# haoyann/koordinator

Measured on AMD Instinct MI355X. Metric: pod-node Filter+Score evals/sec + p99 per-pod sched latency @50k nodes, higher is better.
Workload: dtype int64

## Files before the change

### include/koord_eval.h

```cpp
#ifndef KOORD_EVAL_H
#define KOORD_EVAL_H

#include <stdint.h>

#ifdef __cplusplus
extern "C" {
#endif

#define KE_ABI_VERSION 14
#define KE_ABSENT (-1)

typedef struct ke_ctx ke_ctx;

#define KE_OK 0
#define KE_ERR_INVALID (-1)
#define KE_ERR_UNSUPPORTED (-2)
#define KE_ERR_DEVICE (-3)
#define KE_ERR_NOT_FOUND (-4)
#define KE_ERR_NO_DEVICE (-5)

#define KE_CODE_SUCCESS 0
#define KE_CODE_ERROR 1
#define KE_CODE_UNSCHEDULABLE 2
#define KE_CODE_UNSCHEDULABLE_AND_UNRESOLVABLE 3
// ... 656 lines not shown
int ke_last_kernel_stats(ke_ctx* ctx, double* eval_ms, double* select_ms, double* resolve_ms, int32_t* samples);
int ke_last_kernel_stats_ex(ke_ctx* ctx, double* v8, int32_t* samples, int32_t* pipelined_batches);
int ke_set_pipeline(ke_ctx* ctx, int32_t on);
int ke_last_host_stats(ke_ctx* ctx, double* ms8);
int ke_last_resolve_split(ke_ctx* ctx, double* prologue_ms, double* replay_ms);
int ke_debug_resolve_phases(ke_ctx* ctx, double* phases6);
int ke_debug_resolve_subphases(ke_ctx* ctx, double* sub5);
int ke_debug_resolve_wave1(ke_ctx* ctx, double* w4);
int ke_debug_numa_deferred(ke_ctx* ctx, int64_t* n);
int ke_debug_ds_cuts(ke_ctx* ctx, int32_t* cuts);
int ke_debug_rsv_fused(ke_ctx* ctx, int64_t* out2);
int ke_debug_replay_phases(ke_ctx* ctx, double* cyc8);
int ke_debug_kernel_phases(ke_ctx* ctx, int32_t kernel, double* cyc8);
int ke_debug_spec_failed(ke_ctx* ctx, double* per_batch);
int ke_debug_call_boundary(ke_ctx* ctx, int64_t* out4);
int ke_debug_check_records(ke_ctx* ctx, int64_t now_ns, int64_t* mismatched_nodes);
int ke_bench_eval_kernel(ke_ctx* ctx, int32_t n_pods, const ke_pod* pods, int64_t now_ns, int32_t iters,
                         double* avg_ms);

int ke_row_bytes(void);
int ke_pod_record_bytes(void);
int ke_debug_rows(ke_ctx* ctx, int32_t n, int64_t now_ns, void* device_rows, void* host_rows);
int64_t ke_debug_usage_bound(int64_t total, int64_t thr);
int32_t ke_num_nodes(ke_ctx* ctx);
int ke_debug_node_state(ke_ctx* ctx, int32_t node, ke_node* out, int32_t cpu_cap, ke_cpu* cpus, int32_t* n_cpus,
                        int32_t zone_cap, ke_numa_zone* zones, int32_t* n_zones, int32_t dev_cap, ke_device* devs,
                        int32_t* n_devs);

#ifdef __cplusplus
}
// ... 3 lines not shown
```

### koordinator_amd/abi.py

```python
import ctypes as C
import os

import numpy as np

ABI_VERSION = 14
ABSENT = -1

OK = 0
ERR_INVALID, ERR_UNSUPPORTED, ERR_DEVICE, ERR_NOT_FOUND, ERR_NO_DEVICE = -1, -2, -3, -4, -5

CODE_SUCCESS, CODE_ERROR, CODE_UNSCHEDULABLE, CODE_UNSCHEDULABLE_AND_UNRESOLVABLE, CODE_SKIP = 0, 1, 2, 3, 5

REASON_NONE = 0
REASON_LA_NODEMETRIC_EXPIRED = 1
REASON_LA_USAGE_CPU = 2
REASON_LA_USAGE_MEMORY = 3
REASON_LA_AGG_USAGE_CPU = 4
REASON_LA_AGG_USAGE_MEMORY = 5
REASON_NUMA_INSUFFICIENT_AMPLIFIED_CPU = 16
REASON_NUMA_INVALID_AMPLIFICATION_RATIO = 17
REASON_NUMA_INVALID_CPU_TOPOLOGY = 18
REASON_NUMA_POLICY_CONFLICT = 19
REASON_NUMA_MISSING_RESOURCES = 20
REASON_NUMA_HINT_UNALIGNED = 21
# ... 542 lines not shown
    "ke_last_kernel_stats_ex": (C.c_int, [C.c_void_p, C.c_void_p, C.POINTER(i32), C.POINTER(i32)]),
    "ke_set_pipeline": (C.c_int, [C.c_void_p, i32]),
    "ke_debug_replay_phases": (C.c_int, [C.c_void_p, C.c_void_p]),
    "ke_debug_kernel_phases": (C.c_int, [C.c_void_p, C.c_int32, C.c_void_p]),
    "ke_debug_check_records": (C.c_int, [C.c_void_p, i64, C.POINTER(i64)]),
    "ke_last_host_stats": (C.c_int, [C.c_void_p, C.c_void_p]),
    "ke_last_resolve_split": (C.c_int, [C.c_void_p, C.POINTER(C.c_double), C.POINTER(C.c_double)]),
    "ke_debug_resolve_phases": (C.c_int, [C.c_void_p, C.c_void_p]),
    "ke_debug_resolve_subphases": (C.c_int, [C.c_void_p, C.c_void_p]),
    "ke_debug_resolve_wave1": (C.c_int, [C.c_void_p, C.c_void_p]),
    "ke_debug_numa_deferred": (C.c_int, [C.c_void_p, C.POINTER(i64)]),
    "ke_debug_ds_cuts": (C.c_int, [C.c_void_p, C.POINTER(i32)]),
    "ke_debug_rsv_fused": (C.c_int, [C.c_void_p, C.POINTER(i64)]),
    "ke_debug_spec_failed": (C.c_int, [C.c_void_p, C.POINTER(C.c_double)]),
    "ke_debug_call_boundary": (C.c_int, [C.c_void_p, C.c_void_p]),
    "ke_bench_eval_kernel": (C.c_int, [C.c_void_p, i32, C.c_void_p, i64, i32, C.POINTER(C.c_double)]),
    "ke_row_bytes": (C.c_int, []),
    "ke_pod_record_bytes": (C.c_int, []),
    "ke_debug_rows": (C.c_int, [C.c_void_p, i32, i64, C.c_void_p, C.c_void_p]),
    "ke_debug_usage_bound": (i64, [i64, i64]),
    "ke_num_nodes": (i32, [C.c_void_p]),
    "ke_debug_node_state": (C.c_int, [C.c_void_p, i32, C.c_void_p, i32, C.c_void_p, C.c_void_p, i32, C.c_void_p,
                                      C.c_void_p, i32, C.c_void_p, C.c_void_p]),
    "ke_comm_unique_id": (C.c_int, [C.c_void_p, i32]),
    "ke_shard_init": (C.c_int, [C.c_void_p, i32, i32, C.c_void_p]),
    "ke_shard_init_host": (C.c_int, [C.c_void_p, i32, i32, C.c_void_p, C.c_void_p]),
    "ke_shard_range": (C.c_int, [C.c_void_p, C.POINTER(i32), C.POINTER(i32)]),
}
COMM_ID_BYTES = 128

_lib = None


def load_library(path=LIB_PATH):
    global _lib
    if _lib is not None and path == LIB_PATH:
        return _lib
    if not os.path.exists(path):
        raise RuntimeError(f"{path} is missing: run __graft_entry__.build() (hipcc --offload-arch=gfx950)")
    lib = C.CDLL(path)
    for name, (res, args) in EXPORTS.items():
        fn = getattr(lib, name)
        fn.restype = res
        fn.argtypes = args
    if lib.ke_abi_version() != ABI_VERSION:
        raise RuntimeError("libkoordeval.so ABI version mismatch")
    sizes = (i32 * len(STRUCTS))()
    lib.ke_abi_struct_sizes(sizes, len(STRUCTS))
    for s, n in zip(STRUCTS, sizes):
        if C.sizeof(s) != n:
            raise RuntimeError(f"ABI layout mismatch for {s.__name__}: python {C.sizeof(s)} != C {n}")
    if path == LIB_PATH:
        _lib = lib
    return lib


def ptr(arr):
# ... 17 lines not shown
```

### koordinator_amd/csrc/ke_capi.cpp

```cpp
#include <algorithm>
#include <chrono>
#include <cstring>
#include <deque>
#include <new>

#include "ke_host.h"

namespace ke {
const char* last_error_cstr();
int device_available();
int device_create(Context* ctx);
void device_destroy(Context* ctx);
int device_eval(Context* ctx, int32_t n_pods, const ke_pod* pods, int64_t now, uint8_t* status, uint8_t* reason,
                int16_t* la, int16_t* numa, int16_t* ds, int16_t* total, int32_t* best);
int device_schedule(Context* ctx, int32_t n_pods, const ke_pod* pods, int64_t now, int32_t* chosen, int32_t* score);
int device_rsv_result(Context* ctx, int32_t* out4);
int device_rsv_gate(const Context* ctx);
int device_refresh(Context* ctx, int64_t now, bool defer);
int device_ds_views(Context* ctx, const ke_pod& pod, int64_t now, const std::vector<DsView>& views,
                    std::vector<DsViewOut>& out);
int device_rsv_views(Context* ctx, const ke_pod& pod, int64_t now, const std::vector<RsvView>& views,
                     std::vector<RsvViewOut>& out);
int device_numa_views(Context* ctx, const ke_pod& pod, int64_t now, const std::vector<NumaRsvView>& views,
                      std::vector<NumaRsvOut>& out);
// ... 1534 lines not shown
  return device_replay_phases(&ctx->c, kernel, cyc8);
}

int ke_debug_spec_failed(ke_ctx* ctx, double* per_batch) {
  if (!ctx || !per_batch) return fail(KE_ERR_INVALID, "ke_debug_spec_failed arguments");
  *per_batch = ctx->c.kstat_spec_failed;
  return KE_OK;
}

int ke_debug_call_boundary(ke_ctx* ctx, int64_t* out4) {
  if (!ctx || !out4) return fail(KE_ERR_INVALID, "ke_debug_call_boundary arguments");
  for (int i = 0; i < 4; i++) out4[i] = ctx->c.call_boundary[i];
  return KE_OK;
}

int ke_debug_check_records(ke_ctx* ctx, int64_t now_ns, int64_t* mismatched_nodes) {
  if (ctx) async_drain(ctx);
  if (!ctx || !mismatched_nodes) return fail(KE_ERR_INVALID, "ke_debug_check_records arguments");
  flush_mirror(ctx->c);
  int rc = require_device(ctx);
  if (rc) return rc;
  return device_check_records(&ctx->c, now_ns, mismatched_nodes);
}

int ke_set_pipeline(ke_ctx* ctx, int32_t on) {
  if (ctx) async_drain(ctx);
  if (!ctx) return fail(KE_ERR_INVALID, "null context");
  int rc = require_device(ctx);
  if (rc) return rc;
  return device_set_pipeline(&ctx->c, on);
// ... 121 lines not shown
```

### koordinator_amd/csrc/ke_host.h

```cpp
#pragma once
#include <atomic>
#include <chrono>
#include <cstdint>
#include <functional>
#include <map>
#include <string>
#include <thread>
#include <utility>
#include <vector>

#include "../../include/koord_eval.h"
#include "ke_types.h"

namespace ke {

struct AssignedPod {
  struct {
    int64_t pod_key;
    int64_t custom_seconds_after_scheduled, custom_seconds_after_initialized, initialized_transition_ns;
    int32_t priority_class;
    uint8_t has_initialized;
  } pod;
  int64_t ts;
  int64_t est[KE_NRES];
// ... 85 lines not shown
  bool ext_enabled = false;
  int32_t n_bind_nodes = 0;
  int32_t n_policy_nodes = 0;
  std::vector<uint64_t> last_cpusets;
  std::vector<int64_t> last_numa_alloc;
  std::vector<uint64_t> last_dev_alloc;
  std::vector<int32_t> last_chosen;
  std::vector<int64_t> last_uid;
  std::vector<uint8_t> last_quota;
  DeviceState* dev = nullptr;
  double last_total_ms = 0.0;
  std::vector<double> last_batch_ms;
  double kstat_eval_ms = 0, kstat_select_ms = 0, kstat_resolve_ms = 0, kstat_fixup_ms = 0, kstat_handoff_ms = 0;
  int32_t last_pipelined = 0;
  int64_t call_boundary[4] = {0, 0, 0, 0};
  bool call_behind = false;
  uint64_t prev_end_tick = 0;
  int32_t last_ds_cuts = 0;
  double kstat_spec_failed = 0;
  double kstat_rows_fetched = 0, kstat_rows_changed = 0;
  double last_enqueue_ms = 0;
  double host_ms[8] = {0, 0, 0, 0, 0, 0, 0, 0};
  double kstat_resolve_prologue_ms = 0, kstat_resolve_loop_ms = 0;
  double kstat_resolve_phase_ms[6] = {0, 0, 0, 0, 0, 0};
  double kstat_resolve_sub_ms[5] = {0, 0, 0, 0, 0};
  double kstat_resolve_wave1_ms[4] = {0, 0, 0, 0};
  int64_t kstat_numa_deferred = 0;
  int32_t kstat_samples = 0;
  struct PendingAssign {
    int32_t node;
// ... 171 lines not shown
```

### koordinator_amd/csrc/ke_kernels.hip

```cpp
#include <hip/hip_runtime.h>
#include <rccl/rccl.h>

#include <algorithm>
#include <chrono>
#include <cstdio>
#include <cstdlib>
#include <cstring>
#include <vector>

#include "ke_cpuacc.h"
#include "ke_merge.h"
#include "ke_host.h"
#include "ke_types.h"

namespace ke {

extern "C" __device__ uint32_t __ockl_wfred_max_u32(uint32_t);
extern "C" __device__ int32_t __ockl_wfred_add_i32(int32_t);

#define HIP_OK(expr)                                                                 \
  do {                                                                               \
    hipError_t _e = (expr);                                                          \
    if (_e != hipSuccess) {                                                          \
      return fail(KE_ERR_DEVICE, std::string(#expr ": ") + hipGetErrorString(_e));  \
    }                                                                                \
  } while (0)

constexpr int EVAL_BLOCK = 256;
constexpr int PST = 16;
inline dim3 eval_grid(int n_nodes, int block, int pods, int ppb) {
  const int tiles = (n_nodes + block - 1) / block;
  return dim3((unsigned)((tiles + 7) / 8 * 8), (unsigned)((pods + ppb - 1) / ppb));
}
constexpr int SELECT_BLOCK = 1024;
constexpr int SELECT_WAVES = SELECT_BLOCK / 64;
constexpr int KMAX = MAX_BATCH;

struct SoA {
  int64_t* f;
  uint32_t* flags;
  int64_t stride;
  int64_t* ds;
  uint64_t* dsm;
// ... 2584 lines not shown
  for (int u = 0; u < RW_PAD; u++) w[u] = __hip_atomic_load(const_cast<int64_t*>(rec + u), __ATOMIC_RELAXED, SCOPE);
  w[RW_PAD] = 0;
  rec_unpack(w, f);
}
__device__ __forceinline__ void rec_load_plain(const int64_t* __restrict__ rec, NodeFast& f) {
  int64_t w[NUM_RW];
  const int4* r4 = reinterpret_cast<const int4*>(rec);
#pragma unroll
  for (int u = 0; u < NUM_RW / 2; u++) {
    const int4 q = r4[u];
    w[2 * u] = (int64_t)(((uint64_t)(uint32_t)q.y << 32) | (uint32_t)q.x);
    w[2 * u + 1] = (int64_t)(((uint64_t)(uint32_t)q.w << 32) | (uint32_t)q.z);
  }
  rec_unpack(w, f);
}
__device__ __forceinline__ void rec_unpack(const int64_t (&w)[NUM_RW], NodeFast& f) {
#pragma unroll
  for (int v = 0; v < 2; v++)
#pragma unroll
    for (int q = 0; q < 2; q++) {
      f.fh[v][q] = w[RW_FH + 2 * v + q];
      f.sa[v][q] = __longlong_as_double(w[RW_SA + 2 * v + q]);
    }
#pragma unroll
  for (int q = 0; q < 2; q++) {
    f.cap[q] = __longlong_as_double(w[RW_CAP + q]);
    f.rcap[q] = __longlong_as_double(w[RW_RCAP + q]);
    f.al[q] = __longlong_as_double(w[RW_AL + q]);
    f.ral[q] = __longlong_as_double(w[RW_RAL + q]);
    f.nreq[q] = __longlong_as_double(w[RW_NREQ + q]);
// ... 299 lines not shown
      if ((threadIdx.x & 63) == 0 && m) atomicMax(dsmax1 + p, m);
    } else if (DS) {
      dsraw[(int64_t)p * score_stride + i] = (uint16_t)(o.total >= 0 ? 1u : 0u);
    }
    if (CPU && NUMA) aff_out[i] = o.aff;
  }
}

constexpr int EVAL_PPB = 8;
__host__ __device__ constexpr bool use_record_eval(int pods) { return pods > 2; }
template <bool EXT, int NS = 0>
__global__ __launch_bounds__(EVAL_BLOCK) void k_eval_plain(SoA s, int lo, int hi, const DevPod* __restrict__ pods,
                                                           const int32_t* __restrict__ batch_base, int batch_pods,
                                                           KArgs k, uint16_t* __restrict__ scores, int64_t score_stride,
                                                           uint64_t* __restrict__ stamp, const int32_t* __restrict__ done_wait,
                                                           int32_t* __restrict__ err) {
  if (done_wait) {
    __shared__ int32_t s_go;
    if (threadIdx.x == 0) s_go = wait_at_least(done_wait, 1, err);
    __syncthreads();
    if (!s_go) return;
  }
  if (stamp && (blockIdx.x | blockIdx.y | threadIdx.x) == 0) stamp[0] = __builtin_amdgcn_s_memrealtime();
  const int G = (int)gridDim.y;
  const int b = (int)(blockIdx.x + blockIdx.y * gridDim.x), r = b >> 3;
  const int tile = (r / G) * 8 + (b & 7), group = r % G;
  const int i = lo + tile * blockDim.x + threadIdx.x;
  const int base = *batch_base;
  const int p0 = group * EVAL_PPB;
  const int np = min(batch_pods, p0 + EVAL_PPB) - p0;
  __shared__ double s_pd[EVAL_PPB][4];
  __shared__ int64_t s_pi[EVAL_PPB][3];
  __shared__ uint32_t s_pf[EVAL_PPB];
  __shared__ uint64_t s_ns[NS ? EVAL_PPB : 1][EVAL_BLOCK / 64];
  uint64_t off[2] = {0ull, 0ull};
  if constexpr (NS == NS_SCORES) {
    static_assert(EVAL_PPB == 8, "two words of four offsets");
#pragma unroll
    for (int q = 0; q < EVAL_PPB; q++) {
      const uint16_t v = q < np && i < hi ? s.nsc_tbl[(int64_t)((uint32_t)s.ns_ids[base + p0 + q] >> 16) * s.nsc_stride + i] : (uint16_t)0;
      off[q >> 2] |= (uint64_t)v << ((q & 3) * 16);
    }
  }
  if ((int)threadIdx.x < 4 * np) {
    const int q = threadIdx.x >> 2, c = threadIdx.x & 3;
    const DevPod& pp = pods[base + p0 + q];
    if constexpr (NS) {
      static_assert(EVAL_BLOCK / 64 == 4, "one table word per wave of the block");
      const int w = ((lo + tile * (int)blockDim.x) >> 6) + c;
      const int idw = s.ns_ids[base + p0 + q];
      s_ns[q][c] = w < s.ns_wps ? s.ns_tbl[(int64_t)(NS == NS_SCORES ? idw & 0xffff : idw) * s.ns_wps + w] : 0ull;
    }
    s_pd[q][c] = (double)(c < 2 ? pp.est[c] : pp.req[c - 2]);
    if (!EXT && c < 3) s_pi[q][c] = c < 2 ? pp.est[c] : pp.req[0];
    if (!EXT && c == 3) s_pf[q] = pp.flags;
  }
  __syncthreads();
  if (i >= hi) return;
  NodeFast f;
  rec_load_plain(s.rec + (int64_t)i * NUM_RW, f);
  if (EXT && (k.flags & AF_EXT)) ext_load(s, i, k, f);
  fast_adopt(f, k);
  uint16_t* const out = scores + (int64_t)p0 * score_stride + i;
  for (int q = 0; q < np; q++) {
    const double ed[2] = {s_pd[q][0], s_pd[q][1]}, rd[2] = {s_pd[q][2], s_pd[q][3]};
    int32_t t;
    if constexpr (EXT) {
      t = fast_total<EXT>(f, pods[base + p0 + q], ed, rd, k);
    } else {
      DevPod pl;
      pl.flags = s_pf[q];
      pl.est[0] = s_pi[q][0];
      pl.est[1] = s_pi[q][1];
      pl.req[0] = s_pi[q][2];
      t = fast_total<false>(f, pl, ed, rd, k);
    }
    if constexpr (NS == NS_SCORES) t = t >= 0 ? t + (int32_t)((uint32_t)((q < 4 ? off[0] : off[1]) >> ((q & 3) * 16)) & 0xffffu) : t;
    if (NS && !((s_ns[q][threadIdx.x >> 6] >> (threadIdx.x & 63)) & 1ull)) t = -1;
    out[(int64_t)q * score_stride] = (uint16_t)(t + 1);
  }
}

template <bool EXT, int NS = 0>
__global__ __launch_bounds__(64) void k_patch(SoA s, const DevPod* __restrict__ pods, const int32_t* __restrict__ batch_base,
                                              KArgs k, const int32_t* __restrict__ tlist, uint16_t* __restrict__ scores,
                                              int64_t score_stride, const int32_t* __restrict__ done_wait,
                                              int32_t* __restrict__ err) {
  const int j = blockIdx.x, t = threadIdx.x;
  {
    __shared__ int32_t s_go;
    if (t == 0) s_go = wait_at_least(done_wait, 1, err);
    __syncthreads();
    if (!s_go) return;
  }
  const int n = ld_sc1(tlist);
// ... 3194 lines not shown
    int64_t cpusets_cap = 0;
    int32_t* d_sched = nullptr;
    int64_t sched_cap = 0;
    PinnedVec<uint8_t> h_out;
    std::vector<hipEvent_t> tev;
  } alt;
  uint16_t* d_scores2 = nullptr;
  uint32_t* d_split2 = nullptr;
  uint32_t* d_stale = nullptr;
  uint32_t* d_pre = nullptr;
  uint32_t* d_chg = nullptr;
  int64_t* d_trows = nullptr;
  int32_t* d_tcnt = nullptr;
  int32_t* d_parts_done = nullptr;
  int32_t* d_stale_cnt = nullptr;
  static constexpr int EV_RING = 8;
  hipEvent_t ev_res[EV_RING] = {};
  hipEvent_t ev_sel[EV_RING] = {};
  hipEvent_t ev_start = nullptr;
  hipEvent_t ev_refresh[2] = {};
  bool refresh_pending[2] = {};
  int refresh_cur = 0;
  std::vector<std::function<void(const int32_t*)>> deferred;
  int32_t* d_rsv_gate = nullptr;
  bool refresh_sync = false;
  bool pipeline = true;
  bool pipe_fixup = false;
  unsigned excl_lds = EXCL_LDS;
  bool eval_patch = true;
  bool select_ahead = true;
// ... 83 lines not shown
  HIP_OK(hipMalloc(&d->d_cand, sizeof(uint32_t) * MAX_BATCH * KMAX));
  HIP_OK(hipMalloc(&d->d_cand_cnt, sizeof(int32_t) * MAX_BATCH));
  HIP_OK(hipMalloc(&d->d_batch_base, sizeof(int32_t)));
  HIP_OK(hipMemsetAsync(d->d_batch_base, 0, sizeof(int32_t), d->stream));
  HIP_OK(hipMalloc(&d->d_stale, sizeof(uint32_t) * 2 * MAX_BATCH * KSTALE));
  HIP_OK(hipMalloc(&d->d_pre, sizeof(uint32_t) * 2 * MAX_BATCH * (KSTALE2 + 1)));
  HIP_OK(hipMalloc(&d->d_stale_cnt, sizeof(int32_t) * 2 * MAX_BATCH));
  HIP_OK(hipMalloc(&d->d_trows, sizeof(int64_t) * MAX_BATCH * NUM_RW));
  HIP_OK(hipMalloc(&d->soa.rec, sizeof(int64_t) * NUM_RW * d->capacity));
  HIP_OK(hipMalloc(&d->soa.kerr, sizeof(int32_t)));
  HIP_OK(hipMemsetAsync(d->soa.kerr, 0, sizeof(int32_t), d->stream));
  HIP_OK(hipMemsetAsync(d->soa.rec, 0, sizeof(int64_t) * NUM_RW * d->capacity, d->stream));
  HIP_OK(hipMalloc(&d->d_tcnt, sizeof(int32_t)));
  HIP_OK(hipMalloc(&d->d_parts_done, sizeof(int32_t) * 2 * MAX_BATCH));
  HIP_OK(hipMemset(d->d_parts_done, 0, sizeof(int32_t) * 2 * MAX_BATCH));
  if (d->capacity > (int64_t)CHG_LDS_WORDS * 32) {
    HIP_OK(hipMalloc(&d->d_chg, sizeof(uint32_t) * (d->capacity + 31) / 32));
    HIP_OK(hipMemsetAsync(d->d_chg, 0, sizeof(uint32_t) * (d->capacity + 31) / 32, d->stream));
  }
  HIP_OK(hipMalloc(&d->d_dsraw, sizeof(uint16_t) * MAX_BATCH * d->capacity));
  HIP_OK(hipMalloc(&d->d_dsmax, sizeof(uint32_t) * DSB_WORDS));
  d->soa.dsb = d->d_dsmax;
  d->soa.dsraw = d->d_dsraw;
  HIP_OK(hipMalloc(&d->d_aff, d->capacity));
  HIP_OK(hipMalloc(&d->d_split, sizeof(uint32_t) * GATH_WORDS_MAX * MAX_WORLD));
  HIP_OK(hipMalloc(&d->d_rsv_out, sizeof(int32_t) * 4));
  HIP_OK(hipMalloc(&d->d_rsv_st, sizeof(RsvPickSt)));
  HIP_OK(hipStreamSynchronize(d->stream));
  return KE_OK;
}

int device_refresh(Context* ctx, int64_t now, bool defer = false);
int device_refresh_flush(Context* ctx, const int32_t* gate);
static KArgs make_kargs(const Context* ctx, int64_t now);
int device_rsv_views(Context* ctx, const ke_pod& pod, int64_t now, const std::vector<RsvView>& views,
                     std::vector<RsvViewOut>& out) {
  DeviceState* d = ctx->dev;
  out.assign(views.size(), RsvViewOut{});
  if (views.empty()) return KE_OK;
  HIP_OK(hipSetDevice(d->device));
  int rc = device_refresh(ctx, now);
  if (rc) return rc;
  for (const RsvView& v : views)
    if (v.node < 0 || v.node >= ctx->n_nodes) return fail(KE_ERR_DEVICE, "reservation view node out of range");
// ... 80 lines not shown
  return d->h_rsv_out.size() >= 5 ? d->h_rsv_out[4] : 0;
}

void device_destroy(Context* ctx) {
  DeviceState* d = ctx->dev;
  if (!d) return;
  (void)hipSetDevice(d->device);
  if (d->stream) (void)hipStreamSynchronize(d->stream);
  if (d->comm) (void)ncclCommDestroy(d->comm);
  void* ptrs[] = {d->soa.f,     d->soa.flags, d->d_rows,      d->d_idx,          d->d_pods,   d->d_scores,
                  d->d_cand,    d->d_cand_cnt, d->d_batch_base, d->d_out,
                  d->d_parity, d->d_best,      d->d_gath,    d->d_split,         d->soa.ds,   d->soa.dsm,
                  d->d_dsraw,   d->d_dsmax,  d->d_devalloc,   d->d_dsrows,       d->soa.nf,   d->soa.nm,
                  d->d_numaalloc, d->d_numarows, d->d_defer, d->d_defer_cnt, d->soa.cs, d->soa.cpu,
                  d->d_cpurows, d->d_cpusets, d->d_aff, d->soa.qt, d->soa.qm, d->d_sched, d->d_stale,
                  d->d_stale_cnt, d->d_pre, d->d_trows, d->d_tcnt, d->d_parts_done, d->d_scores2, d->d_split2, d->d_chg, d->soa.rec, d->soa.pt, d->soa.kerr,
                  d->soa.xf, d->soa.xm, d->d_xrows, d->soa.dsx, d->d_ph, d->d_vfo, d->d_rsv, d->d_rsv_out, d->d_rsv_st,
                  d->d_rsv_views, d->d_ds_views, d->d_numa_views, d->d_rovr, d->d_rsv_gate, d->d_ns_tbl, d->d_nsc_tbl};
  if (d->estream) (void)hipStreamSynchronize(d->estream);
  if (d->estream2) (void)hipStreamSynchronize(d->estream2);
  for (void* p : ptrs)
    if (p) (void)hipFree(p);
  for (int e = 0; e < DeviceState::EV_RING; e++) {
    if (d->ev_res[e]) (void)hipEventDestroy(d->ev_res[e]);
    if (d->ev_sel[e]) (void)hipEventDestroy(d->ev_sel[e]);
  }
  if (d->ev_start) (void)hipEventDestroy(d->ev_start);
  for (hipEvent_t e : d->ev_refresh)
    if (e) (void)hipEventDestroy(e);
  if (d->estream) (void)hipStreamDestroy(d->estream);
  if (d->cstream) (void)hipStreamDestroy(d->cstream);
// ... 1012 lines not shown
                        ? (cpu ? (numa ? k_eval_batch<true, true, true, false, true> : k_eval_batch<true, false, true, false, true>)
                               : (numa ? k_eval_batch<true, true, false, false, true> : k_eval_batch<true, false, false, false, true>))
                  : cpu ? (ds ? (numa ? k_eval_batch<true, true, true> : k_eval_batch<true, false, true>)
                              : (numa ? k_eval_batch<false, true, true> : k_eval_batch<false, false, true>))
                        : ds ? (numa ? k_eval_batch<true, true, false> : k_eval_batch<true, false, false>)
                             : (numa ? k_eval_batch<false, true, false>
                                     : ns == NS_SCORES
                                         ? ((k.flags & AF_EXT) ? k_eval_batch<false, false, false, true, false, NS_SCORES>
                                                               : k_eval_batch<false, false, false, false, false, NS_SCORES>)
                                     : ns ? ((k.flags & AF_EXT) ? k_eval_batch<false, false, false, true, false, NS_SETS>
                                                                : k_eval_batch<false, false, false, false, false, NS_SETS>)
                                          : ((k.flags & AF_EXT) ? k_eval_batch<false, false, false, true>
                                                                : k_eval_batch<false, false, false>));
        uint32_t* dcnt = numa ? d->d_defer_cnt + b : nullptr;
        if (plain_rec)
          hipLaunchKernelGGL((ns == NS_SCORES ? ((k.flags & AF_EXT) ? k_eval_plain<true, NS_SCORES> : k_eval_plain<false, NS_SCORES>)
                              : ns ? ((k.flags & AF_EXT) ? k_eval_plain<true, NS_SETS> : k_eval_plain<false, NS_SETS>)
                                 : ((k.flags & AF_EXT) ? k_eval_plain<true> : k_eval_plain<false>)), grid, dim3(eb), 0, es, d->soa,
                             lo, hi, d->d_pods, bbase, bp, k, scores, d->capacity, fold_begin ? estamps + b : nullptr,
                             wait_kernel ? nullptr : dwait, d_err);
        else
          hipLaunchKernelGGL(eval, grid, dim3(eb), 0, es, d->soa, lo, hi, d->d_pods, bbase, bp,
                             ppb, k, scores, d->capacity, d->d_dsraw, d->d_defer, dcnt, d->d_aff, d->d_dsmax,
                             fold_begin ? estamps + b : nullptr);
        if (numa) {
          uint32_t* fb = reinterpret_cast<uint32_t*>(d->d_defer + (int64_t)MAX_BATCH * d->capacity);
          hipLaunchKernelGGL((cpu ? k_numa_fallback<false, true> : k_numa_fallback<false, false>), dim3(FALLBACK_BLOCKS),
                             dim3(64), 0, es, d->soa, d->d_pods,
                             bbase, k, d->d_defer, dcnt, scores, d->capacity, 0, nullptr, nullptr,
                             nullptr, nullptr, nullptr, nullptr, ds ? d->d_dsmax : nullptr, cpu ? d->d_aff : nullptr,
                             ds ? d->d_dsraw : nullptr, fb);
          hipLaunchKernelGGL((cpu ? k_numa_finish<false, true> : k_numa_finish<false, false>), dim3(FINISH_BLOCKS),
                             dim3(64), 0, es, d->soa, d->d_pods,
                             bbase, k, d->d_defer, dcnt, scores, d->capacity, 0, nullptr, nullptr,
                             nullptr, nullptr, nullptr, nullptr, ds ? d->d_dsmax : nullptr, cpu ? d->d_aff : nullptr,
// ... 338 lines not shown
  }
  std::memcpy(&herr, h + o_err, 4);
  std::memcpy(&kerr, h + o_kerr, 4);
  const uint64_t prev_end = ctx->prev_end_tick;
  ctx->prev_end_tick = 0;
  std::memcpy(fst.data(), h + o_fst, 16 * nb);
  std::memcpy(st.data(), h + o_st, 8 * (nb + 1));
  std::memcpy(pst.data(), h + o_pst, 8 * PST * nb);
  std::memcpy(est.data(), h + o_est, 8 * nb);
  ctx->host_ms[5] = ms_since(tp);
  tp = clk::now();
  if (herr) {
    if (d->d_chg)
      (void)hipMemset(d->d_chg, 0, sizeof(uint32_t) * (d->capacity + 31) / 32);
    (void)hipMemset(d->d_parts_done, 0, sizeof(int32_t) * 2 * MAX_BATCH);
    return fail(KE_ERR_DEVICE, "pipelined schedule: a device-side hand-off timed out (placements invalid)");
  }
  if (kerr & (KERR_HINT_ROUTE | KERR_LDS_WAIT)) {
    return fail(KE_ERR_DEVICE, (kerr & KERR_LDS_WAIT) ? "internal: a replay LDS wait expired (placements invalid)"
                                                      : "internal: a hinted pod reached a kernel without the hint path");
  }
  float ms = 0;
  HIP_OK(hipEventElapsedTime(&ms, e0, e1));
  ctx->last_total_ms = ms;
  ctx->last_pipelined = n_pipelined;
  const double span = (double)(st[n_batches] - st[0]);
  const double ms_per_tick = span > 0 ? ms / span : 1e-5;
  ctx->call_boundary[0] = 0;
  ctx->call_boundary[1] = cb_copies;
  ctx->call_boundary[2] = cb_fills;
// ... 149 lines not shown
  DeviceState* d = ctx->dev;
  HIP_OK(hipSetDevice(d->device));
  if (n_pods < 1 || n_pods > MAX_BATCH || iters < 1) return fail(KE_ERR_INVALID, "bench: 1 <= n_pods <= 64, iters >= 1");
  int rc = device_refresh(ctx, now);
  if (rc) return rc;
  rc = upload_pods(ctx, n_pods, pods);
  if (rc) return rc;
  const int N = ctx->n_nodes;
  if (N == 0) return fail(KE_ERR_INVALID, "bench: no nodes");
  const KArgs k = make_kargs(ctx, now);
  const int ppb = EVAL_PPB;
  HIP_OK(hipMemsetAsync(d->d_batch_base, 0, sizeof(int32_t), d->stream));
  const dim3 grid = eval_grid(N, EVAL_BLOCK, n_pods, ppb);
  auto launch = [&]() {
    if (use_record_eval(n_pods))
      hipLaunchKernelGGL((k_eval_plain<false>), grid, dim3(EVAL_BLOCK), 0, d->stream, d->soa, 0, N, d->d_pods,
                         d->d_batch_base, n_pods, k, d->d_scores, d->capacity, nullptr, nullptr, nullptr);
    else
      hipLaunchKernelGGL((k_eval_batch<false, false, false>), grid, dim3(EVAL_BLOCK), 0, d->stream, d->soa, 0, N,
                         d->d_pods, d->d_batch_base, n_pods, ppb, k, d->d_scores, d->capacity, d->d_dsraw, d->d_defer,
                         nullptr, d->d_aff, d->d_dsmax, nullptr);
  };
  launch();
  hipEvent_t e0, e1;
  HIP_OK(hipEventCreate(&e0));
  HIP_OK(hipEventCreate(&e1));
  HIP_OK(hipEventRecord(e0, d->stream));
  for (int it = 0; it < iters; it++) launch();
  HIP_OK(hipGetLastError());
  HIP_OK(hipEventRecord(e1, d->stream));
  HIP_OK(hipEventSynchronize(e1));
  float ms = 0;
// ... 55 lines not shown
```

### koordinator_amd/csrc/ke_types.h

```cpp
#pragma once
#include <stdint.h>

#if defined(__HIPCC__) || defined(__HIP__)
#define KE_HD __host__ __device__
#else
#define KE_HD
#endif

namespace ke {

enum RowField : int {
  F_UT = 0,
  F_FH = 1,
  F_SA = 5,
  F_CAP = 9,
  F_NALLOC = 11,
  F_NREQ = 13,
  F_CSM = 15,
  F_CSAF = 16,
  F_CSAS = 17,
  NUM_I64_FIELDS = 18
};

enum NodeFlag : uint32_t {
// ... 306 lines not shown
constexpr int XF_ALLOC = 0, XF_REQ = NUM_XS, XF_PODS = 2 * NUM_XS, NUM_XF = 2 * NUM_XS + 1;

constexpr uint32_t KEY_IDX_BITS = 22;
constexpr uint32_t KEY_IDX_MASK = (1u << KEY_IDX_BITS) - 1;
constexpr int MAX_SHARD_NODES = (1 << KEY_IDX_BITS) - 1;
constexpr int MAX_TOTAL_SCORE = 1022;
constexpr int MAX_DS_RAW = 300;
KE_HD inline uint32_t make_key(int32_t total, int32_t idx) {
  return total < 0 ? 0u : ((uint32_t)(total + 1) << KEY_IDX_BITS) | (KEY_IDX_MASK - (uint32_t)idx);
}
KE_HD inline int32_t key_node(uint32_t key) { return (int32_t)(KEY_IDX_MASK - (key & KEY_IDX_MASK)); }
KE_HD inline int32_t key_score(uint32_t key) { return (int32_t)(key >> KEY_IDX_BITS) - 1; }

constexpr int MAX_BATCH = 64;

}
```

### koordinator_amd/evaluator.py

```python
import ctypes as C

import numpy as np

from . import abi


class KoordEvalError(RuntimeError):
    def __init__(self, code, msg):
        super().__init__(f"koord-eval error {code}: {msg}")
        self.code = code


def pack_node_sets(sets, n_nodes=None):
    if isinstance(sets, np.ndarray) and sets.ndim == 2:
        m = np.ascontiguousarray(sets, dtype=bool)
    else:
        idx = [np.asarray(x, np.int64).reshape(-1) for x in sets]
        if n_nodes is None:
            n_nodes = max([int(x.max()) + 1 for x in idx if len(x)], default=0)
        m = np.zeros((len(idx), n_nodes), bool)
        for r, x in enumerate(idx):
            if len(x) and (x.min() < 0 or x.max() >= n_nodes):
                raise ValueError("node index outside 0..n_nodes")
            m[r, x] = True
# ... 436 lines not shown
        return {"eval_ms": ms4[0], "select_ms": ms4[1], "fixup_ms": ms4[2], "resolve_ms": ms4[3], "samples": n.value,
                "pipelined_batches": npipe.value, "enqueue_ms": ms4[4], "handoff_ms": ms4[5],
                "rows_fetched": ms4[6], "rows_changed": ms4[7], "spec_failed_rounds": sf.value,
                "resolve_prologue_ms": p.value, "resolve_replay_ms": r.value,
                "resolve_phases_ms": dict(zip(["prologue", "spec_predict", "spec_reserve_eval", "spec_verify", "spec_later_rounds", "writeback",
                                               "sub_t_setup", "sub_predict_loop", "sub_t_rows_wave1", "sub_reserve_R",
                                               "t_helper_hit"],
                                              ph.tolist() + sub.tolist())),
                "resolve_wave1_ms": dict(zip(["wait", "reserve", "rows", "end"], w1.tolist()))}

    def call_boundary(self):
        out = np.zeros(4, np.int64)
        self._check(self.lib.ke_debug_call_boundary(self.h, abi.ptr(out)))
        return dict(zip(("primed_batches", "reserve_stream_copies", "reserve_stream_fills", "boundary_ns"), out.tolist()))

    def bench_eval_kernel(self, pods, now_ns, iters):
        pods = as_pod_array(pods)
        ms = C.c_double()
        self._check(self.lib.ke_bench_eval_kernel(self.h, len(pods), abi.ptr(pods), int(now_ns), iters, C.byref(ms)))
        return ms.value

    def node_state(self, i):
        return abi.node_state(self.lib.ke_debug_node_state, self.h, i)

    def debug_rows(self, now_ns, device=True):
        n = self.num_nodes
        host = np.zeros(n, abi.ROW_DTYPE)
        dev = np.zeros(n, abi.ROW_DTYPE) if device else None
        self._check(self.lib.ke_debug_rows(self.h, n, int(now_ns), abi.ptr(dev), abi.ptr(host)))
        return dev, host


def comm_unique_id(lib=None):
    lib = lib or abi.load_library()
    buf = C.create_string_buffer(abi.COMM_ID_BYTES)
    rc = lib.ke_comm_unique_id(buf, abi.COMM_ID_BYTES)
    if rc != abi.OK:
        raise KoordEvalError(rc, lib.ke_last_error().decode())
    return buf.raw
```

Before: 20.62 billion.

## Make plain eval kernel persistent with atomic work-stealing over tile-pod chunks

Replaces the fixed 2D grid of the record-based eval kernel with an occupancy-sized persistent grid. Each block pulls (tile, pod-range) chunks from per-class atomic counters, and all batch pods are staged in LDS once per block. The aim is to cut tail imbalance and launch/over-subscription cost at large node counts, and to reuse each node record across more pods per load. The cost is atomic traffic, counter reset logic, extra syncthreads for namespace tables, and an unused wave-cooperative record loader. Debug plan/slot APIs are also added.

```diff
diff --git a/include/koord_eval.h b/include/koord_eval.h
--- a/include/koord_eval.h
+++ b/include/koord_eval.h
@@ -694,6 +694,8 @@
 int ke_debug_kernel_phases(ke_ctx* ctx, int32_t kernel, double* cyc8);
 int ke_debug_spec_failed(ke_ctx* ctx, double* per_batch);
 int ke_debug_call_boundary(ke_ctx* ctx, int64_t* out4);
+int ke_debug_eval_plan(int32_t n_nodes, int32_t n_pods, int32_t slots, int32_t* out8, int32_t* cover);
+int ke_debug_eval_slots(ke_ctx* ctx, int32_t* slots);
 int ke_debug_check_records(ke_ctx* ctx, int64_t now_ns, int64_t* mismatched_nodes);
 int ke_bench_eval_kernel(ke_ctx* ctx, int32_t n_pods, const ke_pod* pods, int64_t now_ns, int32_t iters,
                          double* avg_ms);
diff --git a/koordinator_amd/abi.py b/koordinator_amd/abi.py
--- a/koordinator_amd/abi.py
+++ b/koordinator_amd/abi.py
@@ -580,6 +580,8 @@
     "ke_debug_rsv_fused": (C.c_int, [C.c_void_p, C.POINTER(i64)]),
     "ke_debug_spec_failed": (C.c_int, [C.c_void_p, C.POINTER(C.c_double)]),
     "ke_debug_call_boundary": (C.c_int, [C.c_void_p, C.c_void_p]),
+    "ke_debug_eval_plan": (C.c_int, [i32, i32, i32, C.c_void_p, C.c_void_p]),
+    "ke_debug_eval_slots": (C.c_int, [C.c_void_p, C.POINTER(i32)]),
     "ke_bench_eval_kernel": (C.c_int, [C.c_void_p, i32, C.c_void_p, i64, i32, C.POINTER(C.c_double)]),
     "ke_row_bytes": (C.c_int, []),
     "ke_pod_record_bytes": (C.c_int, []),
@@ -606,7 +608,11 @@
         raise RuntimeError(f"{path} is missing: run __graft_entry__.build() (hipcc --offload-arch=gfx950)")
     lib = C.CDLL(path)
     for name, (res, args) in EXPORTS.items():
-        fn = getattr(lib, name)
+        fn = getattr(lib, name, None)
+        if fn is None and "KOORDEVAL_LIB" in os.environ and name.startswith("ke_debug_"):
+            continue
+        if fn is None:
+            raise RuntimeError(f"{path} does not export {name}")
         fn.restype = res
         fn.argtypes = args
     if lib.ke_abi_version() != ABI_VERSION:
diff --git a/koordinator_amd/csrc/ke_capi.cpp b/koordinator_amd/csrc/ke_capi.cpp
--- a/koordinator_amd/csrc/ke_capi.cpp
+++ b/koordinator_amd/csrc/ke_capi.cpp
@@ -1572,6 +1572,36 @@
   return KE_OK;
 }
 
+int ke_debug_eval_slots(ke_ctx* ctx, int32_t* slots) {
+  if (!ctx || !slots) return fail(KE_ERR_INVALID, "ke_debug_eval_slots arguments");
+  *slots = ctx->c.eval_slots;
+  return KE_OK;
+}
+
+int ke_debug_eval_plan(int32_t n_nodes, int32_t n_pods, int32_t slots, int32_t* out8, int32_t* cover) {
+  if (!out8 || n_nodes < 1 || n_pods < 1 || n_pods > MAX_BATCH || slots < 1)
+    return fail(KE_ERR_INVALID, "ke_debug_eval_plan arguments");
+  const EvalPlan p = eval_plan(n_nodes, n_pods, slots);
+  const int32_t o[8] = {p.blocks, p.chunk, p.items, p.max_items, p.max_pairs, p.classes, p.tiles, EVAL_TILE};
+  for (int i = 0; i < 8; i++) out8[i] = o[i];
+  if (cover) {
+    for (int c = 0; c < p.classes; c++) {
+      const int pairs = eval_class_pairs(p.tiles, p.classes, c, n_pods);
+      for (int a0 = 0; a0 < pairs; a0 += p.chunk) {
+        const int e = std::min(a0 + p.chunk, pairs);
+        for (int a = a0; a < e;) {
+          int p0, p1;
+          const int tile = eval_segment(a, e, n_pods, p.classes, c, &p0, &p1);
+          if (tile < 0 || tile >= p.tiles || p1 <= p0) return fail(KE_ERR_INVALID, "ke_debug_eval_plan: an item leaves the tiles");
+          for (int q = p0; q < p1; q++) cover[(int64_t)tile * n_pods + q]++;
+          a += p1 - p0;
+        }
+      }
+    }
+  }
+  return KE_OK;
+}
+
 int ke_debug_check_records(ke_ctx* ctx, int64_t now_ns, int64_t* mismatched_nodes) {
   if (ctx) async_drain(ctx);
   if (!ctx || !mismatched_nodes) return fail(KE_ERR_INVALID, "ke_debug_check_records arguments");
diff --git a/koordinator_amd/csrc/ke_host.h b/koordinator_amd/csrc/ke_host.h
--- a/koordinator_amd/csrc/ke_host.h
+++ b/koordinator_amd/csrc/ke_host.h
@@ -123,6 +123,7 @@
   double kstat_eval_ms = 0, kstat_select_ms = 0, kstat_resolve_ms = 0, kstat_fixup_ms = 0, kstat_handoff_ms = 0;
   int32_t last_pipelined = 0;
   int64_t call_boundary[4] = {0, 0, 0, 0};
+  int32_t eval_slots = 0;
   bool call_behind = false;
   uint64_t prev_end_tick = 0;
   int32_t last_ds_cuts = 0;
diff --git a/koordinator_amd/csrc/ke_kernels.hip b/koordinator_amd/csrc/ke_kernels.hip
--- a/koordinator_amd/csrc/ke_kernels.hip
+++ b/koordinator_amd/csrc/ke_kernels.hip
@@ -27,6 +27,7 @@
   } while (0)
 
 constexpr int EVAL_BLOCK = 256;
+constexpr int EVAL_CTR_STRIDE = 32;
 constexpr int PST = 16;
 inline dim3 eval_grid(int n_nodes, int block, int pods, int ppb) {
   const int tiles = (n_nodes + block - 1) / block;
@@ -2641,6 +2642,42 @@
   }
   rec_unpack(w, f);
 }
+constexpr int REC_HALF = 32 * NUM_RW / 2;
+__device__ __forceinline__ void rec_load_wave(const int64_t* __restrict__ rec, int n_valid, int4* buf, NodeFast& f) {
+  static_assert(NUM_RW == 26, "13 16-byte words a record");
+  const int lane = (int)(threadIdx.x & 63);
+  const int4* g = reinterpret_cast<const int4*>(rec);
+  const int n4 = n_valid * (NUM_RW / 2);
+  int64_t w[NUM_RW];
+#pragma unroll
+  for (int h = 0; h < 2; h++) {
+    __builtin_amdgcn_sched_barrier(0);
+    int4 v[7];
+#pragma unroll
+    for (int j = 0; j < 7; j++) {
+      const int x = lane + 64 * j;
+      v[j] = (x < REC_HALF && h * REC_HALF + x < n4) ? g[h * REC_HALF + x] : make_int4(0, 0, 0, 0);
+    }
+    __builtin_amdgcn_fence(__ATOMIC_RELEASE, "wavefront");
+    __builtin_amdgcn_wave_barrier();
+#pragma unroll
+    for (int j = 0; j < 7; j++) {
+      const int x = lane + 64 * j;
+      if (x < REC_HALF) buf[x] = v[j];
+    }
+    __builtin_amdgcn_fence(__ATOMIC_ACQ_REL, "wavefront");
+    __builtin_amdgcn_wave_barrier();
+    if (h == 0 || lane >= 32) {
+#pragma unroll
+      for (int u = 0; u < NUM_RW / 2; u++) {
+        const int4 q = buf[(lane & 31) * (NUM_RW / 2) + u];
+        w[2 * u] = (int64_t)(((uint64_t)(uint32_t)q.y << 32) | (uint32_t)q.x);
+        w[2 * u + 1] = (int64_t)(((uint64_t)(uint32_t)q.w << 32) | (uint32_t)q.z);
+      }
+    }
+  }
+  rec_unpack(w, f);
+}
 __device__ __forceinline__ void rec_unpack(const int64_t (&w)[NUM_RW], NodeFast& f) {
 #pragma unroll
   for (int v = 0; v < 2; v++)
@@ -2970,71 +3007,117 @@
                                                            const int32_t* __restrict__ batch_base, int batch_pods,
                                                            KArgs k, uint16_t* __restrict__ scores, int64_t score_stride,
                                                            uint64_t* __restrict__ stamp, const int32_t* __restrict__ done_wait,
-                                                           int32_t* __restrict__ err) {
+                                                           int32_t* __restrict__ err, int32_t* __restrict__ ctr, int classes,
+                                                           int chunk) {
+  static_assert(EVAL_BLOCK == EVAL_TILE && EVAL_BLOCK >= 4 * MAX_BATCH, "a lane per node of a tile; four lanes stage a pod");
+  __shared__ int32_t s_go, s_item[2];
+  bool go = true;
   if (done_wait) {
-    __shared__ int32_t s_go;
     if (threadIdx.x == 0) s_go = wait_at_least(done_wait, 1, err);
     __syncthreads();
-    if (!s_go) return;
-  }
-  if (stamp && (blockIdx.x | blockIdx.y | threadIdx.x) == 0) stamp[0] = __builtin_amdgcn_s_memrealtime();
-  const int G = (int)gridDim.y;
-  const int b = (int)(blockIdx.x + blockIdx.y * gridDim.x), r = b >> 3;
-  const int tile = (r / G) * 8 + (b & 7), group = r % G;
-  const int i = lo + tile * blockDim.x + threadIdx.x;
+    go = s_go != 0;
+  }
+  if (stamp && (blockIdx.x | threadIdx.x) == 0) stamp[0] = __builtin_amdgcn_s_memrealtime();
   const int base = *batch_base;
-  const int p0 = group * EVAL_PPB;
-  const int np = min(batch_pods, p0 + EVAL_PPB) - p0;
-  __shared__ double s_pd[EVAL_PPB][4];
-  __shared__ int64_t s_pi[EVAL_PPB][3];
-  __shared__ uint32_t s_pf[EVAL_PPB];
+  __shared__ double s_pd[MAX_BATCH][4];
+  __shared__ int64_t s_pi[MAX_BATCH][3];
+  __shared__ uint32_t s_pf[MAX_BATCH];
   __shared__ uint64_t s_ns[NS ? EVAL_PPB : 1][EVAL_BLOCK / 64];
-  uint64_t off[2] = {0ull, 0ull};
-  if constexpr (NS == NS_SCORES) {
-    static_assert(EVAL_PPB == 8, "two words of four offsets");
-#pragma unroll
-    for (int q = 0; q < EVAL_PPB; q++) {
-      const uint16_t v = q < np && i < hi ? s.nsc_tbl[(int64_t)((uint32_t)s.ns_ids[base + p0 + q] >> 16) * s.nsc_stride + i] : (uint16_t)0;
-      off[q >> 2] |= (uint64_t)v << ((q & 3) * 16);
-    }
-  }
-  if ((int)threadIdx.x < 4 * np) {
+  if ((int)threadIdx.x < 4 * batch_pods) {
     const int q = threadIdx.x >> 2, c = threadIdx.x & 3;
-    const DevPod& pp = pods[base + p0 + q];
-    if constexpr (NS) {
-      static_assert(EVAL_BLOCK / 64 == 4, "one table word per wave of the block");
-      const int w = ((lo + tile * (int)blockDim.x) >> 6) + c;
-      const int idw = s.ns_ids[base + p0 + q];
-      s_ns[q][c] = w < s.ns_wps ? s.ns_tbl[(int64_t)(NS == NS_SCORES ? idw & 0xffff : idw) * s.ns_wps + w] : 0ull;
-    }
+    const DevPod& pp = pods[base + q];
     s_pd[q][c] = (double)(c < 2 ? pp.est[c] : pp.req[c - 2]);
     if (!EXT && c < 3) s_pi[q][c] = c < 2 ? pp.est[c] : pp.req[0];
     if (!EXT && c == 3) s_pf[q] = pp.flags;
   }
+  const int cls = (int)blockIdx.x % classes, wgs = (int)gridDim.x / classes;
+  const int pairs = eval_class_pairs((hi - lo + EVAL_TILE - 1) / EVAL_TILE, classes, cls, batch_pods);
+  const int items = (pairs + chunk - 1) / chunk;
   __syncthreads();
-  if (i >= hi) return;
-  NodeFast f;
-  rec_load_plain(s.rec + (int64_t)i * NUM_RW, f);
-  if (EXT && (k.flags & AF_EXT)) ext_load(s, i, k, f);
-  fast_adopt(f, k);
-  uint16_t* const out = scores + (int64_t)p0 * score_stride + i;
-  for (int q = 0; q < np; q++) {
-    const double ed[2] = {s_pd[q][0], s_pd[q][1]}, rd[2] = {s_pd[q][2], s_pd[q][3]};
-    int32_t t;
-    if constexpr (EXT) {
-      t = fast_total<EXT>(f, pods[base + p0 + q], ed, rd, k);
-    } else {
-      DevPod pl;
-      pl.flags = s_pf[q];
-      pl.est[0] = s_pi[q][0];
-      pl.est[1] = s_pi[q][1];
-      pl.req[0] = s_pi[q][2];
-      t = fast_total<false>(f, pl, ed, rd, k);
-    }
-    if constexpr (NS == NS_SCORES) t = t >= 0 ? t + (int32_t)((uint32_t)((q < 4 ? off[0] : off[1]) >> ((q & 3) * 16)) & 0xffffu) : t;
-    if (NS && !((s_ns[q][threadIdx.x >> 6] >> (threadIdx.x & 63)) & 1ull)) t = -1;
-    out[(int64_t)q * score_stride] = (uint16_t)(t + 1);
-  }
+  int t = (int)blockIdx.x / classes;
+  for (int par = 0;; par ^= 1) {
+    int32_t nxt = 0;
+    bool claimed = false;
+    const int e = t < items && go ? min(t * chunk + chunk, pairs) : 0;
+    for (int a = t * chunk; a < e;) {
+      int p0, p1;
+      const int tile = eval_segment(a, e, batch_pods, classes, cls, &p0, &p1);
+      a += p1 - p0;
+      const int i0 = lo + tile * EVAL_TILE + (int)(threadIdx.x & ~63u);
+      const int i = i0 + (int)(threadIdx.x & 63);
+      const bool live = i < hi;
+      NodeFast f;
+      if (live) rec_load_plain(s.rec + (int64_t)i * NUM_RW, f);
+      if (!claimed && threadIdx.x == 0)
+        nxt = __hip_atomic_fetch_add(ctr + cls * EVAL_CTR_STRIDE, 1, __ATOMIC_RELAXED, __HIP_MEMORY_SCOPE_AGENT);
+      claimed = true;
+      if (live) {
+        if (EXT && (k.flags & AF_EXT)) ext_load(s, i, k, f);
+        fast_adopt(f, k);
+      }
+      constexpr int ROUND = NS ? EVAL_PPB : MAX_BATCH;
+      for (int g0 = p0; g0 < p1; g0 += ROUND) {
+        const int np = min(p1 - g0, ROUND);
+        uint64_t off[2] = {0ull, 0ull};
+        if constexpr (NS == NS_SCORES) {
+          static_assert(EVAL_PPB == 8, "two words of four offsets");
+#pragma unroll
+          for (int q = 0; q < EVAL_PPB; q++) {
+            const uint16_t v = q < np && live ? s.nsc_tbl[(int64_t)((uint32_t)s.ns_ids[base + g0 + q] >> 16) * s.nsc_stride + i] : (uint16_t)0;
+            off[q >> 2] |= (uint64_t)v << ((q & 3) * 16);
+          }
+        }
+        if constexpr (NS) {
+          static_assert(EVAL_BLOCK / 64 == 4, "one table word per wave of the block");
+          __syncthreads();
+          if ((int)threadIdx.x < 4 * np) {
+            const int q = threadIdx.x >> 2, c = threadIdx.x & 3;
+            const int w = ((lo + tile * EVAL_TILE) >> 6) + c;
+            const int idw = s.ns_ids[base + g0 + q];
+            s_ns[q][c] = w < s.ns_wps ? s.ns_tbl[(int64_t)(NS == NS_SCORES ? idw & 0xffff : idw) * s.ns_wps + w] : 0ull;
+          }
+          __syncthreads();
+        }
+        if (!live) continue;
+        uint16_t* const out = scores + (int64_t)g0 * score_stride + i;
+        for (int q = 0; q < np; q++) {
+          const double ed[2] = {s_pd[g0 + q][0], s_pd[g0 + q][1]}, rd[2] = {s_pd[g0 + q][2], s_pd[g0 + q][3]};
+          int32_t t2;
+          if constexpr (EXT) {
+            t2 = fast_total<EXT>(f, pods[base + g0 + q], ed, rd, k);
+          } else {
+            DevPod pl;
+            pl.flags = s_pf[g0 + q];
+            pl.est[0] = s_pi[g0 + q][0];
+            pl.est[1] = s_pi[g0 + q][1];
+            pl.req[0] = s_pi[g0 + q][2];
+            t2 = fast_total<false>(f, pl, ed, rd, k);
+          }
+          if constexpr (NS == NS_SCORES) t2 = t2 >= 0 ? t2 + (int32_t)((uint32_t)((q < 4 ? off[0] : off[1]) >> ((q & 3) * 16)) & 0xffffu) : t2;
+          if (NS && !((s_ns[q][threadIdx.x >> 6] >> (threadIdx.x & 63)) & 1ull)) t2 = -1;
+          out[(int64_t)q * score_stride] = (uint16_t)(t2 + 1);
+        }
+      }
+    }
+    if (threadIdx.x == 0) {
+      if (!claimed) nxt = __hip_atomic_fetch_add(ctr + cls * EVAL_CTR_STRIDE, 1, __ATOMIC_RELAXED, __HIP_MEMORY_SCOPE_AGENT);
+      if (nxt == max(items - wgs, 0) + wgs - 1)
+        __hip_atomic_store(ctr + cls * EVAL_CTR_STRIDE, 0, __ATOMIC_RELAXED, __HIP_MEMORY_SCOPE_AGENT);
+      s_item[par] = nxt;
+    }
+    __syncthreads();
+    const int next = wgs + s_item[par];
+    if (t >= items || next >= items) break;
+    t = next;
+  }
+}
+
+using EvalPlainFn = void (*)(SoA, int, int, const DevPod*, const int32_t*, int, KArgs, uint16_t*, int64_t, uint64_t*,
+                             const int32_t*, int32_t*, int32_t*, int, int);
+inline EvalPlainFn eval_plain_kernel(bool ext, int ns) {
+  return ns == NS_SCORES ? (ext ? k_eval_plain<true, NS_SCORES> : k_eval_plain<false, NS_SCORES>)
+         : ns            ? (ext ? k_eval_plain<true, NS_SETS> : k_eval_plain<false, NS_SETS>)
+                         : (ext ? k_eval_plain<true> : k_eval_plain<false>);
 }
 
 template <bool EXT, int NS = 0>
@@ -6259,6 +6342,8 @@
   int32_t* d_tcnt = nullptr;
   int32_t* d_parts_done = nullptr;
   int32_t* d_stale_cnt = nullptr;
+  int32_t* d_eval_ctr = nullptr;
+  int eval_slots[2][3] = {};
   static constexpr int EV_RING = 8;
   hipEvent_t ev_res[EV_RING] = {};
   hipEvent_t ev_sel[EV_RING] = {};
@@ -6372,6 +6457,21 @@
   HIP_OK(hipMalloc(&d->d_tcnt, sizeof(int32_t)));
   HIP_OK(hipMalloc(&d->d_parts_done, sizeof(int32_t) * 2 * MAX_BATCH));
   HIP_OK(hipMemset(d->d_parts_done, 0, sizeof(int32_t) * 2 * MAX_BATCH));
+  HIP_OK(hipMalloc(&d->d_eval_ctr, sizeof(int32_t) * 2 * 8 * EVAL_CTR_STRIDE));
+  HIP_OK(hipMemset(d->d_eval_ctr, 0, sizeof(int32_t) * 2 * 8 * EVAL_CTR_STRIDE));
+  {
+    int cus = 0, cap = 0;
+    HIP_OK(hipDeviceGetAttribute(&cus, hipDeviceAttributeMultiprocessorCount, d->device));
+    if (const char* e = std::getenv("KOORDEVAL_EVAL_SLOTS")) cap = std::max(1, std::atoi(e));
+    for (int x = 0; x < 2; x++)
+      for (int ns = 0; ns < 3; ns++) {
+        int per_cu = 0;
+        HIP_OK(hipOccupancyMaxActiveBlocksPerMultiprocessor(&per_cu, eval_plain_kernel(x != 0, ns), EVAL_BLOCK, 0));
+        d->eval_slots[x][ns] = std::max(1, per_cu * cus);
+        if (cap) d->eval_slots[x][ns] = std::min(d->eval_slots[x][ns], cap);
+      }
+    ctx->eval_slots = d->eval_slots[0][0];
+  }
   if (d->capacity > (int64_t)CHG_LDS_WORDS * 32) {
     HIP_OK(hipMalloc(&d->d_chg, sizeof(uint32_t) * (d->capacity + 31) / 32));
     HIP_OK(hipMemsetAsync(d->d_chg, 0, sizeof(uint32_t) * (d->capacity + 31) / 32, d->stream));
@@ -6386,6 +6486,15 @@
   HIP_OK(hipMalloc(&d->d_rsv_st, sizeof(RsvPickSt)));
   HIP_OK(hipStreamSynchronize(d->stream));
   return KE_OK;
+}
+
+static void launch_eval_plain(DeviceState* d, hipStream_t es, bool alt, bool ext, int ns, int lo, int hi,
+                              const int32_t* bbase, int bp, const KArgs& k, uint16_t* scores, uint64_t* stamp,
+                              const int32_t* dwait, int32_t* err) {
+  const EvalPlan p = eval_plan(hi - lo, bp, d->eval_slots[ext ? 1 : 0][ns]);
+  hipLaunchKernelGGL(eval_plain_kernel(ext, ns), dim3((unsigned)p.blocks), dim3(EVAL_BLOCK), 0, es, d->soa, lo, hi, d->d_pods,
+                     bbase, bp, k, scores, d->capacity, stamp, dwait, err,
+                     d->d_eval_ctr + (alt ? 8 * EVAL_CTR_STRIDE : 0), p.classes, p.chunk);
 }
 
 int device_refresh(Context* ctx, int64_t now, bool defer = false);
@@ -6496,7 +6605,7 @@
                   d->d_dsraw,   d->d_dsmax,  d->d_devalloc,   d->d_dsrows,       d->soa.nf,   d->soa.nm,
                   d->d_numaalloc, d->d_numarows, d->d_defer, d->d_defer_cnt, d->soa.cs, d->soa.cpu,
                   d->d_cpurows, d->d_cpusets, d->d_aff, d->soa.qt, d->soa.qm, d->d_sched, d->d_stale,
-                  d->d_stale_cnt, d->d_pre, d->d_trows, d->d_tcnt, d->d_parts_done, d->d_scores2, d->d_split2, d->d_chg, d->soa.rec, d->soa.pt, d->soa.kerr,
+                  d->d_stale_cnt, d->d_pre, d->d_trows, d->d_tcnt, d->d_parts_done, d->d_eval_ctr, d->d_scores2, d->d_split2, d->d_chg, d->soa.rec, d->soa.pt, d->soa.kerr,
                   d->soa.xf, d->soa.xm, d->d_xrows, d->soa.dsx, d->d_ph, d->d_vfo, d->d_rsv, d->d_rsv_out, d->d_rsv_st,
                   d->d_rsv_views, d->d_ds_views, d->d_numa_views, d->d_rovr, d->d_rsv_gate, d->d_ns_tbl, d->d_nsc_tbl};
   if (d->estream) (void)hipStreamSynchronize(d->estream);
@@ -7539,11 +7648,8 @@
                                                                 : k_eval_batch<false, false, false>));
         uint32_t* dcnt = numa ? d->d_defer_cnt + b : nullptr;
         if (plain_rec)
-          hipLaunchKernelGGL((ns == NS_SCORES ? ((k.flags & AF_EXT) ? k_eval_plain<true, NS_SCORES> : k_eval_plain<false, NS_SCORES>)
-                              : ns ? ((k.flags & AF_EXT) ? k_eval_plain<true, NS_SETS> : k_eval_plain<false, NS_SETS>)
-                                 : ((k.flags & AF_EXT) ? k_eval_plain<true> : k_eval_plain<false>)), grid, dim3(eb), 0, es, d->soa,
-                             lo, hi, d->d_pods, bbase, bp, k, scores, d->capacity, fold_begin ? estamps + b : nullptr,
-                             wait_kernel ? nullptr : dwait, d_err);
+          launch_eval_plain(d, es, alt, (k.flags & AF_EXT) != 0, ns, lo, hi, bbase, bp, k, scores,
+                            fold_begin ? estamps + b : nullptr, wait_kernel ? nullptr : dwait, d_err);
         else
           hipLaunchKernelGGL(eval, grid, dim3(eb), 0, es, d->soa, lo, hi, d->d_pods, bbase, bp,
                              ppb, k, scores, d->capacity, d->d_dsraw, d->d_defer, dcnt, d->d_aff, d->d_dsmax,
@@ -7912,6 +8018,7 @@
     if (d->d_chg)
       (void)hipMemset(d->d_chg, 0, sizeof(uint32_t) * (d->capacity + 31) / 32);
     (void)hipMemset(d->d_parts_done, 0, sizeof(int32_t) * 2 * MAX_BATCH);
+    (void)hipMemset(d->d_eval_ctr, 0, sizeof(int32_t) * 2 * 8 * EVAL_CTR_STRIDE);
     return fail(KE_ERR_DEVICE, "pipelined schedule: a device-side hand-off timed out (placements invalid)");
   }
   if (kerr & (KERR_HINT_ROUTE | KERR_LDS_WAIT)) {
@@ -8091,8 +8198,8 @@
   const dim3 grid = eval_grid(N, EVAL_BLOCK, n_pods, ppb);
   auto launch = [&]() {
     if (use_record_eval(n_pods))
-      hipLaunchKernelGGL((k_eval_plain<false>), grid, dim3(EVAL_BLOCK), 0, d->stream, d->soa, 0, N, d->d_pods,
-                         d->d_batch_base, n_pods, k, d->d_scores, d->capacity, nullptr, nullptr, nullptr);
+      launch_eval_plain(d, d->stream, false, false, 0, 0, N, d->d_batch_base, n_pods, k, d->d_scores, nullptr, nullptr,
+                        nullptr);
     else
       hipLaunchKernelGGL((k_eval_batch<false, false, false>), grid, dim3(EVAL_BLOCK), 0, d->stream, d->soa, 0, N,
                          d->d_pods, d->d_batch_base, n_pods, ppb, k, d->d_scores, d->capacity, d->d_dsraw, d->d_defer,
diff --git a/koordinator_amd/csrc/ke_types.h b/koordinator_amd/csrc/ke_types.h
--- a/koordinator_amd/csrc/ke_types.h
+++ b/koordinator_amd/csrc/ke_types.h
@@ -344,4 +344,48 @@
 
 constexpr int MAX_BATCH = 64;
 
-}
+constexpr int EVAL_TILE = 256;
+#ifndef KE_EVAL_PASSES
+#define KE_EVAL_PASSES 2
+#endif
+constexpr int EVAL_PASSES = KE_EVAL_PASSES;
+struct EvalPlan {
+  int32_t tiles;
+  int32_t classes;
+  int32_t chunk;
+  int32_t blocks;
+  int32_t items;
+  int32_t max_items;
+  int32_t max_pairs;
+};
+KE_HD inline int eval_class_tiles(int tiles, int classes, int c) { return (tiles - c + classes - 1) / classes; }
+KE_HD inline int eval_class_pairs(int tiles, int classes, int c, int pods) { return eval_class_tiles(tiles, classes, c) * pods; }
+KE_HD inline int eval_segment(int a, int e, int pods, int classes, int c, int* p0, int* p1) {
+  const int lt = a / pods;
+  *p0 = a - lt * pods;
+  *p1 = (e - a) < (pods - *p0) ? *p0 + (e - a) : pods;
+  return lt * classes + c;
+}
+inline EvalPlan eval_plan(int n_nodes, int pods, int slots) {
+  EvalPlan p = {};
+  if (n_nodes < 1 || pods < 1) return p;
+  if (slots < 1) slots = 1;
+  p.tiles = (n_nodes + EVAL_TILE - 1) / EVAL_TILE;
+  p.classes = slots < 8 ? slots : 8;
+  if (p.classes > p.tiles) p.classes = p.tiles;
+  const int per_class = slots / p.classes;
+  const int64_t most = (int64_t)eval_class_pairs(p.tiles, p.classes, 0, pods);
+  int64_t chunk = (most + (int64_t)per_class * EVAL_PASSES - 1) / ((int64_t)per_class * EVAL_PASSES);
+  if (chunk > pods) chunk = pods;
+  p.chunk = (int32_t)chunk;
+  const int64_t most_items = (most + chunk - 1) / chunk;
+  const int bc = (int)(most_items < per_class ? most_items : per_class);
+  p.blocks = bc * p.classes;
+  for (int c = 0; c < p.classes; c++) p.items += (eval_class_pairs(p.tiles, p.classes, c, pods) + p.chunk - 1) / p.chunk;
+  p.max_items = (int32_t)((most_items + bc - 1) / bc);
+  const int64_t mp = (int64_t)p.max_items * chunk;
+  p.max_pairs = (int32_t)(mp < most ? mp : most);
+  return p;
+}
+
+}
diff --git a/koordinator_amd/evaluator.py b/koordinator_amd/evaluator.py
--- a/koordinator_amd/evaluator.py
+++ b/koordinator_amd/evaluator.py
@@ -474,6 +474,11 @@
         self._check(self.lib.ke_debug_call_boundary(self.h, abi.ptr(out)))
         return dict(zip(("primed_batches", "reserve_stream_copies", "reserve_stream_fills", "boundary_ns"), out.tolist()))
 
+    def eval_slots(self):
+        n = C.c_int32()
+        self._check(self.lib.ke_debug_eval_slots(self.h, C.byref(n)))
+        return n.value
+
     def bench_eval_kernel(self, pods, now_ns, iters):
         pods = as_pod_array(pods)
         ms = C.c_double()
@@ -489,6 +494,22 @@
         dev = np.zeros(n, abi.ROW_DTYPE) if device else None
         self._check(self.lib.ke_debug_rows(self.h, n, int(now_ns), abi.ptr(dev), abi.ptr(host)))
         return dev, host
+
+
+EVAL_PLAN_FIELDS = ("blocks", "pairs_per_item", "items", "max_items", "max_pairs", "classes", "tiles", "tile_nodes")
+
+
+def eval_plan(n_nodes, n_pods, slots, cover=False, lib=None):
+    lib = lib or abi.load_library()
+    out = np.zeros(8, np.int32)
+    cov = np.zeros(((int(n_nodes) + 255) // 256, int(n_pods)), np.int32) if cover else None
+    rc = lib.ke_debug_eval_plan(int(n_nodes), int(n_pods), int(slots), abi.ptr(out), abi.ptr(cov))
+    if rc != abi.OK:
+        raise KoordEvalError(rc, lib.ke_last_error().decode())
+    plan = dict(zip(EVAL_PLAN_FIELDS, out.tolist()))
+    if cover:
+        plan["cover"] = cov
+    return plan
 
 
 def comm_unique_id(lib=None):
```

After: 19.53 billion. -5.3%, worse.
